# patrickltobing/cyclevae-vc

Measured on AMD Instinct MI355X. Metric: mcep_frames_per_sec_hu1024_ld32_cyc2, higher is better.
Workload: dtype f32 (every matrix product on exact fp32 operands: each operand carried as three fp16 limbs x = l0 + l1/2^11 + l2/2^22, six v_mfma_f32_32x32x16_f16 per product, f32 accumulate; dropped terms < 2^-33 of a product; gates, carried state, projection and outputs f32)

## Files before the change

cyclevae-vc_amd/csrc/cvae_exact3.h:

```cpp
#pragma once
#include <cvae_intrin.h>

struct Step6Params {
    const float* gx0;
    const float* w2s;
    float* hbuf;
    long mtot;
    float* hx;
    const float* wrec3;
    const float* afold3;
    const float* cfold;
    const float* bhn;
    const float* xt;
    int Tp, Cp;
    int B, Bp, H, T;
    unsigned* flags;
    int* status;
    long long* prof;
    const float* wyT;
    const float* dy;
    int Co;
    int rts;
    int want_f32;
    int exp;
    int backoff;
    const float* gx;
    long gx_bstride;
};

__global__ void k_prep_wrec3(const float* wrec2, float* wrec3, int H, int KPW, int* unfit) {
    const int nch = H >> 4, NB = H >> 3;
    const long idx = (long)blockIdx.x * blockDim.x + threadIdx.x;
    if (idx < (long)NB * 4 * KPW * 512) {
        const int e = (int)(idx & 7), lane = (int)((idx >> 3) & 63);
        const int s = (int)((idx >> 9) % KPW), wave = (int)(((idx >> 9) / KPW) & 3), c = (int)((idx >> 9) / KPW / 4);
        const int col = lane & 31, kh = lane >> 5, g = col >> 3, u = col & 7, j = 8 * c + u;
        const int k = 16 * (wave * KPW + s) + 8 * kh + e;
        float w = 0.0f;
        if (k < H) w = wrec2[((((long)(j >> 4) * 4 + g) * nch + (k >> 4)) * 16 + (j & 15)) * 16 + (k & 15)];
        unsigned short l0, l1, l2;
        cvae_split3_f16(w, l0, l1, l2);
        cvae_flag_unfit(unfit, w);
        unsigned short* dst = (unsigned short*)wrec3 + ((((long)c * 4 + wave) * KPW + s) * 3) * 512 + lane * 8 + e;
        dst[0] = l0;
        dst[512] = l1;
        dst[1024] = l2;
    }
}

__global__ void k_prep_wrec3_l2b(const float* wrec2, unsigned char* w2s, int H, int KPW) {
    const int nch = H >> 4, NB = H >> 3;
    const long idx = (long)blockIdx.x * blockDim.x + threadIdx.x;
    if (idx < (long)NB * 4 * KPW * 512) {
        const int e = (int)(idx & 7), lane = (int)((idx >> 3) & 63);
        const int s = (int)((idx >> 9) % KPW), wave = (int)(((idx >> 9) / KPW) & 3), c = (int)((idx >> 9) / KPW / 4);
        const int col = lane & 31, kh = lane >> 5, g = col >> 3, u = col & 7, j = 8 * c + u;
        const int k = 16 * (wave * KPW + s) + 8 * kh + e;
        float w = 0.0f;
        if (k < H) w = wrec2[((((long)(j >> 4) * 4 + g) * nch + (k >> 4)) * 16 + (j & 15)) * 16 + (k & 15)];
        unsigned short l0, l1;
        unsigned char l2;
        cvae_split3_f16b8(w, l0, l1, l2);
        w2s[idx] = l2;
    }
}

__global__ void k_prep_afold3l(const float* afold, float* afold3, int H, int Kfe, int KFW, int* unfit) {
    const int NB = H >> 3;
    const long idx = (long)blockIdx.x * blockDim.x + threadIdx.x;
    if (idx < (long)NB * 4 * KFW * 512) {
        const int e = (int)(idx & 7), lane = (int)((idx >> 3) & 63);
        const int s = (int)((idx >> 9) % KFW), wave = (int)(((idx >> 9) / KFW) & 3), c = (int)((idx >> 9) / KFW / 4);
        const int col = lane & 31, kh = lane >> 5, g = col >> 3, u = col & 7;
        const int k = 16 * (wave * KFW + s) + 8 * kh + e;
        const float w = (g < 3 && k < Kfe) ? afold[(long)(g * H + 8 * c + u) * Kfe + k] : 0.0f;
        unsigned short l0, l1, l2;
        cvae_split3_f16(w, l0, l1, l2);
        cvae_flag_unfit(unfit, w);
        unsigned short* dst = (unsigned short*)afold3 + ((((long)c * 4 + wave) * KFW + s) * 3) * 512 + lane * 8 + e;
        dst[0] = l0;
        dst[512] = l1;
        dst[1024] = l2;
    }
}

__device__ __forceinline__ f32x16 cvae_zero16() {
    f32x16 z;
#pragma unroll
    for (int q = 0; q < 16; ++q) z[q] = 0.0f;
    return z;
}

template <int KPW, int KFW, int LIMBS = 3, bool W2S = false>
__global__ __launch_bounds__(256, 1) void k_gru_steps_v6(Step6Params p) {
    constexpr int RS = 40;
    constexpr float S1 = 1.0f / 2048.0f;
#ifndef CVAE_V6_RD
#define CVAE_V6_RD 8
#endif
    constexpr int RD0 = W2S ? 5 : CVAE_V6_RD;
    constexpr int RD = KPW < RD0 ? KPW : RD0;
    constexpr bool HOIST = KFW == 0;
    constexpr int RF = HOIST ? 1 : (W2S && KFW > 3 ? 3 : KFW);
    constexpr int RW = KPW < 4 ? KPW : 4;
    const int tid = threadIdx.x, wave = cvae_uniform(tid >> 6), lane = tid & 63, lc = lane & 31, kh = lane >> 5;
    const int H = p.H, NB = H >> 3, nrt = p.Bp >> 5;
    const int rts = p.rts;
    int c, ti;
    cvae_block_map((int)blockIdx.x, NB, rts, (p.exp & 2) != 0, c, ti);
    const int s_lo = wave * KPW;
    float* red = (float*)CVAE_SMEM;
    float* hsh = red + 4 * 32 * RS;
    unsigned short* hl = (unsigned short*)(hsh + 32 * 8);
    float* wfl = hsh + 32 * 8 + 384;
    const int row = tid >> 3, u = tid & 7, j = 8 * c + u;
    const unsigned mtot = (unsigned)p.mtot;
    const cvae_buf hb = cvae_make_buf(p.hbuf, (unsigned)((long)(H >> 4) * p.mtot * 64));
    const cvae_buf xb_ = cvae_make_buf(p.hx, (unsigned)((long)(H >> 4) * p.mtot * 80));
    const unsigned tstride = mtot >> 5;
    const unsigned voff = (unsigned)kh * 512u + (unsigned)lc * 16u, voff2 = 2048u + (unsigned)kh * 256u + (unsigned)lc * 8u;
    f32x4 w0[KPW], w1[KPW], w2[LIMBS == 3 && !W2S ? KPW : 1];
#pragma unroll
    for (int s = 0; s < KPW; ++s) {
        const float* src = p.wrec3 + ((((long)c * 4 + wave) * KPW + s) * 3) * 256 + lane * 4;
        w0[s] = *(const f32x4*)src;
        w1[s] = *(const f32x4*)(src + 256);
        if constexpr (LIMBS == 3 && !W2S) w2[s] = *(const f32x4*)(src + 512);
    }
    {
        const float* src = p.afold3 + ((long)c * 4 + wave) * (KFW * 3 * 256);
        float* dst = wfl + wave * (KFW * LIMBS * 256);
#pragma unroll
        for (int s = 0; s < KFW; ++s)
#pragma unroll
            for (int m = 0; m < LIMBS; ++m)
                *(f32x4*)(dst + (s * LIMBS + m) * 256 + lane * 4) = *(const f32x4*)(src + (s * 3 + m) * 256 + lane * 4);
    }
    __syncthreads();
    const float* wfw = wfl + wave * (KFW * LIMBS * 256) + lane * 4;
    const float bhn = p.bhn[j];
    const float cf0 = HOIST ? 0.f : p.cfold[j], cf1 = HOIST ? 0.f : p.cfold[H + j], cf2 = HOIST ? 0.f : p.cfold[2 * H + j];
    const int ntile = ti < nrt ? (nrt - ti + rts - 1) / rts : 0, ntask = p.T * ntile;
    long long pc[4] = {0, 0, 0, 0};
    f32x4 x4[2 * RF];
    f32x2 x2[RF];
    const unsigned char* xw = nullptr;
    auto set_x = [&](int k) {
        const int tt = k / ntile, ii = ti + (k % ntile) * rts;
        xw = (const unsigned char*)p.xt + (((long)ii * p.Tp + tt) * (p.Cp >> 3) + 2 * (wave * KFW) + kh) * 1280;
    };
    auto load_x = [&](int s) {
        x4[2 * (s % RF)] = *(const f32x4*)(xw + s * 2560 + lc * 16);
        x4[2 * (s % RF) + 1] = *(const f32x4*)(xw + s * 2560 + 512 + lc * 16);
        if constexpr (LIMBS == 3) x2[s % RF] = *(const f32x2*)(xw + s * 2560 + 1024 + lc * 8);
    };
    float gq0 = 0.f, gq1 = 0.f, gq2 = 0.f;
    auto load_g = [&](int k) {
        const int tt = k / ntile, gr = (ti + (k % ntile) * rts) * 32 + row;
        if (gr < p.B) {
            const float* g = p.gx + (long)gr * p.gx_bstride + (long)tt * 3 * H + j;
            gq0 = g[0]; gq1 = g[H]; gq2 = g[2 * H];
        }
    };
    float hkeep0 = 0.f, hkeep1 = 0.f;
    const int backoff = (p.exp >> 8) ? (p.exp >> 8) - 1 : p.backoff;
    if constexpr (HOIST) {
        if (ntask > 0) load_g(0);
    } else if (ntask > 0) {
        set_x(0);
#pragma unroll
        for (int s = 0; s < RF; ++s) load_x(s);
    }
    unsigned fpre = 0u;
    for (int k = 0; k < ntask; ++k) {
        long long c0 = !W2S && p.prof ? cvae_clock() : 0;
        const int t = k / ntile, i = ti + (k % ntile) * rts;
        const unsigned row0 = (unsigned)(t * p.Bp + i * 32), tile0 = row0 >> 5;
        f32x16 a0 = cvae_zero16(), a1 = cvae_zero16(), a2 = cvae_zero16(), a3 = cvae_zero16();
#pragma unroll
        for (int s = 0; s < KFW; ++s) {
            const f32x4 l0 = x4[2 * (s % RF)], l1 = x4[2 * (s % RF) + 1];
            const f32x4 b0 = *(const f32x4*)(wfw + (s * LIMBS + 0) * 256);
            const f32x4 b1 = *(const f32x4*)(wfw + (s * LIMBS + 1) * 256);
            a0 = cvae_mfma_32x32x16_f16(l0, b0, a0);
            a1 = cvae_mfma_32x32x16_f16(l0, b1, a1);
            if constexpr (LIMBS == 3) {
                const f32x4 l2 = cvae_bf8x8_to_h8(x2[s % RF]);
                const f32x4 b2 = *(const f32x4*)(wfw + (s * LIMBS + 2) * 256);
                a2 = cvae_mfma_32x32x16_f16(l1, b1, a2);
                if constexpr (W2S) a2 = cvae_mfma_32x32x16_f16(l0, b2, a2);
                else a3 = cvae_mfma_32x32x16_f16(l0, b2, a3);
                a1 = cvae_mfma_32x32x16_f16(l1, b0, a1);
                a2 = cvae_mfma_32x32x16_f16(l2, b0, a2);
            } else {
                a2 = cvae_mfma_32x32x16_f16(l1, b0, a2);
            }
            cvae_sched_fence();
            if (s + RF < KFW) load_x(s + RF);
        }
        if (!W2S && p.prof) { const long long c1 = cvae_clock(); pc[0] += c1 - c0; c0 = c1; }
        const bool pre_ok = ntile > 1 && k > 0 && cvae_wave_all(fpre >= (unsigned)t);
        if (t > 0 && !pre_ok) {
            unsigned spins = 0;
            if (ntile == 1)
                for (int q = 0; q < backoff; ++q) cvae_sleep_64();
            for (;;) {
                unsigned f = (unsigned)t;
                if (lane < 2 * KPW && 2 * s_lo + lane < NB) f = cvae_atomic_load_agent(p.flags + (long)i * NB + 2 * s_lo + lane);
                if (cvae_wave_all(f >= (unsigned)t)) break;
                cvae_sleep();
                if (++spins > (1u << 22)) {
                    p.status[0] = 2;
                    break;
                }
            }
        }
        cvae_compiler_fence();
        if (!W2S && p.prof) { const long long c1 = cvae_clock(); pc[1] += c1 - c0; c0 = c1; }
        const int grow = i * 32 + row;
        const bool live = grow < p.B;
        const bool keep1 = ntile == 2 && (k & 1);
        float gxr = HOIST ? gq0 : cf0, gxz = HOIST ? gq1 : cf1, gxn = HOIST ? gq2 : cf2, hold = keep1 ? hkeep1 : hkeep0;
        auto gate_inputs = [&]() {
            if (live) {
                if (t == 0 && p.gx0) {
                    const float* g0p = p.gx0 + (long)grow * 3 * H + j;
                    gxr += g0p[0]; gxz += g0p[H]; gxn += g0p[2 * H];
                } else if (t == 0 && p.dy) cvae_t0_fix(p.wyT, p.dy, p.Co, H, j, grow, gxr, gxz, gxn);
                if (t == 0) {
                    hold = cvae_buf_load_f1_sc1(hb, (unsigned)(row * 64 + (j & 15) * 4), ((unsigned)(j >> 4) * mtot + row0) * 64u);
                } else if (ntile > 2) {
                    const unsigned so = ((unsigned)(j >> 4) * tstride + tile0) * 2560u, okh = (unsigned)((j >> 3) & 1);
                    const unsigned vo = okh * 512u + (unsigned)(row * 16 + (u >> 1) * 4);
                    const int sh = (u & 1) * 16;
                    const unsigned q0 = __builtin_bit_cast(unsigned, cvae_buf_load_f1_sc1(xb_, vo, so));
                    const unsigned q1 = __builtin_bit_cast(unsigned, cvae_buf_load_f1_sc1(xb_, vo, so + 1024u));
                    float third = 0.0f;
                    if constexpr (LIMBS == 3) {
                        const unsigned q2 = __builtin_bit_cast(unsigned, cvae_buf_load_f1_sc1(xb_, 2048u + okh * 256u + (unsigned)(row * 8 + (u >> 2) * 4), so));
                        third = cvae_bf8_to_f32((unsigned char)(q2 >> ((u & 3) * 8))) * (S1 / CVAE_L2_SCALE);
                    }
                    hold = cvae_f16_bits_to_f32((unsigned short)(q0 >> sh)) + (cvae_f16_bits_to_f32((unsigned short)(q1 >> sh)) + third) * S1;
                }
            }
        };
        if constexpr (KPW >= 32) gate_inputs();
        f32x4 hc[2 * RD];
        f32x2 hb2[RD];
        const unsigned tsel = (p.exp & 1) ? (unsigned)i : tile0;
        auto load_h = [&](int s) {
            const unsigned so = ((unsigned)(s_lo + s) * tstride + tsel) * 2560u;
            hc[2 * (s % RD)] = cvae_buf_load_f4(xb_, voff, so);
            hc[2 * (s % RD) + 1] = cvae_buf_load_f4(xb_, voff, so + 1024u);
            if constexpr (LIMBS == 3) hb2[s % RD] = cvae_buf_load_f2(xb_, voff2, so);
        };
        f32x2 w2r[W2S ? RW : 1];
        const float* w2base = W2S ? p.w2s + ((long)c * 4 + wave) * KPW * 128 + lane * 2 : nullptr;
        auto load_w2 = [&](int s) { w2r[s % RW] = *(const f32x2*)(w2base + s * 128); };
        if constexpr (W2S) {
#pragma unroll
            for (int s = 0; s < RW; ++s) load_w2(s);
        }
#pragma unroll
        for (int s = 0; s < RD; ++s) load_h(s);
        if constexpr (KPW < 32) gate_inputs();
#pragma unroll
        for (int s = 0; s < KPW; ++s) {
            const f32x4 l0 = hc[2 * (s % RD)], l1 = hc[2 * (s % RD) + 1];
            a0 = cvae_mfma_32x32x16_f16(l0, w0[s], a0);
            a1 = cvae_mfma_32x32x16_f16(l0, w1[s], a1);
            if constexpr (LIMBS == 3) {
                const f32x4 l2 = cvae_bf8x8_to_h8(hb2[s % RD]);
                a2 = cvae_mfma_32x32x16_f16(l1, w1[s], a2);
                if constexpr (W2S) a2 = cvae_mfma_32x32x16_f16(l0, cvae_bf8x8_to_h8(w2r[s % RW]), a2);
                else a3 = cvae_mfma_32x32x16_f16(l0, w2[s], a3);
                a1 = cvae_mfma_32x32x16_f16(l1, w0[s], a1);
                a2 = cvae_mfma_32x32x16_f16(l2, w0[s], a2);
            } else {
                a2 = cvae_mfma_32x32x16_f16(l1, w0[s], a2);
            }
            cvae_sched_fence();
            if (s + RD < KPW) load_h(s + RD);
            if constexpr (W2S) { if (s + RW < KPW) load_w2(s + RW); }
        }
        cvae_sched_fence();
        const int xmode = HOIST ? 0 : (p.exp >> 5) & 3;
        if constexpr (HOIST) {
            if (k + 1 < ntask) load_g(k + 1);
        } else {
            if (k + 1 < ntask) set_x(k + 1);
            if (k + 1 < ntask && (xmode == 0 || (xmode == 2 && wave != 0))) {
#pragma unroll
                for (int s = 0; s < RF; ++s) load_x(s);
            }
        }
#pragma unroll
        for (int q = 0; q < 16; ++q)
            red[(wave * 32 + (q & 3) + 8 * (q >> 2) + 4 * kh) * RS + lc] =
                LIMBS == 3 ? a0[q] + (a1[q] + (a2[q] + a3[q]) * S1) * S1 : a0[q] + (a1[q] + a2[q]) * S1;
        if (!W2S && p.prof) { const long long c1 = cvae_clock(); pc[2] += c1 - c0; c0 = c1; }
        __syncthreads();
        {
            float hn_ = 0.0f;
            if (live) {
                float sg[4];
#pragma unroll
                for (int g = 0; g < 4; ++g)
                    sg[g] = red[(0 * 32 + row) * RS + g * 8 + u] + red[(1 * 32 + row) * RS + g * 8 + u] +
                            red[(2 * 32 + row) * RS + g * 8 + u] + red[(3 * 32 + row) * RS + g * 8 + u];
                const float rg = cvae_sigmoid_fast(gxr + sg[0]);
                const float zg = cvae_sigmoid_fast(gxz + sg[1]);
                const float ng = cvae_tanh_fast(gxn + sg[2] + rg * (sg[3] + bhn));
                hn_ = ng + zg * (hold - ng);
            }
            if (keep1) hkeep1 = hn_; else hkeep0 = hn_;
            hsh[row * 8 + u] = hn_;
            unsigned short l0, l1;
            unsigned char l2;
            cvae_split3_f16b8(hn_, l0, l1, l2);
            hl[row * 8 + u] = l0;
            hl[256 + row * 8 + u] = l1;
            ((unsigned char*)(hl + 512))[row * 8 + u] = l2;
        }
        __syncthreads();
        if (tid < 64) {
            const unsigned so = ((unsigned)(c >> 1) * tstride + tile0 + (unsigned)(p.Bp >> 5)) * 2560u;
            cvae_buf_store_f4_sc1(xb_, (unsigned)(c & 1) * 512u + (unsigned)(tid & 31) * 16u, so + (unsigned)(tid >> 5) * 1024u,
                                  *(const f32x4*)(hl + tid * 8));
            if (LIMBS == 3 && tid < 32)
                cvae_buf_store_f2_sc1(xb_, 2048u + (unsigned)(c & 1) * 256u + (unsigned)tid * 8u, so, *(const f32x2*)(hl + 512 + tid * 4));
            cvae_drain_vmem();
            cvae_wave_barrier();
            if (tid == 0) cvae_atomic_store_agent(p.flags + (long)i * NB + c, (unsigned)(t + 1));
        } else if (tid < 128 && p.want_f32) {
            const int l = tid - 64, r = l >> 1, half = l & 1;
            *(f32x4*)(p.hbuf + (((long)(c >> 1) * p.mtot + row0 + p.Bp + r) * 16 + (c & 1) * 8 + half * 4)) =
                *(const f32x4*)(hsh + r * 8 + half * 4);
        }
        if constexpr (!HOIST) {
            if (k + 1 < ntask && (xmode == 1 || (xmode == 2 && wave == 0))) {
#pragma unroll
                for (int s = 0; s < RF; ++s) load_x(s);
            }
        }
        if (ntile > 1 && k + 1 < ntask) {
            const int kn = k + 1, tn = kn / ntile, in_ = ti + (kn % ntile) * rts;
            fpre = (unsigned)tn;
            if (tn > 0 && lane < 2 * KPW && 2 * s_lo + lane < NB)
                fpre = cvae_atomic_load_agent(p.flags + (long)in_ * NB + 2 * s_lo + lane);
        }
        if (!W2S && p.prof) { const long long c1 = cvae_clock(); pc[3] += c1 - c0; c0 = c1; }
    }
    if (p.prof && tid == 64 * ((p.exp >> 2) & 3))
        for (int q = 0; q < 4; ++q) p.prof[(long)blockIdx.x * 4 + q] = pc[q];
}

struct Out6Params {
    const float* hx;
    long mtot;
    const float* wo3;
    const float* bo2;
    int H, Bp, T, B, ncell, Co, clamp_from;
    float clamp_min;
    float* out[CVAE_MAX_CELLS];
};

__global__ void k_prep_wo3(const float* wo2, float* wo3, int H, int Cop, int NT, int* unfit) {
    const int nk = H >> 4;
    const long idx = (long)blockIdx.x * blockDim.x + threadIdx.x;
    if (idx < (long)NT * nk * 512) {
        const int e = (int)(idx & 7), lane = (int)((idx >> 3) & 63), s = (int)((idx >> 9) % nk), n = (int)((idx >> 9) / nk);
        const int col = 32 * n + (lane & 31), k = 16 * s + 8 * (lane >> 5) + e;
        const float w = col < Cop ? wo2[(long)col * H + k] : 0.0f;
        unsigned short l0, l1, l2;
        cvae_split3_f16(w, l0, l1, l2);
        cvae_flag_unfit(unfit, w);
        unsigned short* dst = (unsigned short*)wo3 + (((long)n * nk + s) * 3) * 512 + lane * 8 + e;
        dst[0] = l0;
        dst[512] = l1;
        dst[1024] = l2;
    }
}

template <int KPW>
__global__ __launch_bounds__(256) void k_outproj_v6(Out6Params p) {
    constexpr float S1 = 1.0f / 2048.0f;
    constexpr int RS = 36;
    const int tid = threadIdx.x, wave = cvae_uniform(tid >> 6), lane = tid & 63, lc = lane & 31, kh = lane >> 5;
    const int nk = p.H >> 4, nt32 = p.Bp >> 5;
    const int n = blockIdx.y;
    const long tile = (long)nt32 + blockIdx.x;
    float* red = (float*)CVAE_SMEM;
    const long tstride = p.mtot >> 5;
    f32x16 a0 = cvae_zero16(), a1 = cvae_zero16(), a2 = cvae_zero16(), a3 = cvae_zero16();
    constexpr int RD = KPW < 4 ? KPW : 4;
    f32x4 ha[2 * RD], wb[3 * RD];
    f32x2 hb[RD];
    auto load = [&](int s) {
        const int sg = wave * KPW + s;
        const unsigned char* hp = (const unsigned char*)p.hx + ((long)sg * tstride + tile) * 2560;
        ha[2 * (s % RD)] = *(const f32x4*)(hp + kh * 512 + lc * 16);
        ha[2 * (s % RD) + 1] = *(const f32x4*)(hp + 1024 + kh * 512 + lc * 16);
        hb[s % RD] = *(const f32x2*)(hp + 2048 + kh * 256 + lc * 8);
        const float* wp = p.wo3 + (((long)n * nk + sg) * 3) * 256 + lane * 4;
#pragma unroll
        for (int m = 0; m < 3; ++m) wb[3 * (s % RD) + m] = *(const f32x4*)(wp + m * 256);
    };
    const bool has_k = wave * KPW < nk;
    if (has_k) {
#pragma unroll
        for (int s = 0; s < RD; ++s) load(s);
#pragma unroll
        for (int s = 0; s < KPW; ++s) {
            const f32x4 l0 = ha[2 * (s % RD)], l1 = ha[2 * (s % RD) + 1], l2 = cvae_bf8x8_to_h8(hb[s % RD]);
            const f32x4 w0 = wb[3 * (s % RD)], w1 = wb[3 * (s % RD) + 1], w2 = wb[3 * (s % RD) + 2];
            a0 = cvae_mfma_32x32x16_f16(l0, w0, a0);
            a1 = cvae_mfma_32x32x16_f16(l0, w1, a1);
            a2 = cvae_mfma_32x32x16_f16(l1, w1, a2);
            a3 = cvae_mfma_32x32x16_f16(l0, w2, a3);
            a1 = cvae_mfma_32x32x16_f16(l1, w0, a1);
            a2 = cvae_mfma_32x32x16_f16(l2, w0, a2);
            cvae_sched_fence();
            if (s + RD < KPW) load(s + RD);
        }
    }
#pragma unroll
    for (int q = 0; q < 16; ++q)
        red[(wave * 32 + (q & 3) + 8 * (q >> 2) + 4 * kh) * RS + lc] = a0[q] + (a1[q] + (a2[q] + a3[q]) * S1) * S1;
    __syncthreads();
    {
        const int r = tid >> 3;
        const long m = (long)blockIdx.x * 32 + r;
        const int t = (int)(m / p.Bp), b = (int)(m - (long)t * p.Bp);
        if (b < p.ncell * p.B) {
            const int cell = b / p.B, bb = b - cell * p.B;
            float* orow = p.out[cell] + ((long)bb * p.T + t) * p.Co;
#pragma unroll
            for (int jj = 0; jj < 4; ++jj) {
                const int cl = (tid & 7) + 8 * jj, col = 32 * n + cl;
                if (col < p.Co) {
                    float v = red[(0 * 32 + r) * RS + cl] + red[(1 * 32 + r) * RS + cl] + red[(2 * 32 + r) * RS + cl] +
                              red[(3 * 32 + r) * RS + cl] + p.bo2[col];
                    if (p.clamp_from >= 0 && col >= p.clamp_from) v = fmaxf(v, p.clamp_min);
                    orow[col] = v;
                }
            }
        }
    }
}

__global__ void k_selftest_occupy(long long cycles, int lds_words) {
    float* occupy_lds = (float*)CVAE_SMEM;
    for (int i = threadIdx.x; i < lds_words; i += blockDim.x) occupy_lds[i] = (float)i;
    __syncthreads();
    const long long t0 = cvae_clock();
    float acc = 0.f;
    int guard = 0;
    while (cvae_clock() - t0 < cycles && ++guard < (1 << 28)) {
        acc += occupy_lds[(threadIdx.x * 33 + guard) % (lds_words > 0 ? lds_words : 1)];
        cvae_sleep();
    }
    if (acc == -1.0f) occupy_lds[0] = acc;
}

__global__ void k_selftest_limbs(const float* x, float* y, long n) {
    const long i0 = 8 * ((long)blockIdx.x * blockDim.x + threadIdx.x);
    if (i0 + 8 > n) return;
    unsigned short l0[8], l1[8];
    unsigned char b[8];
#pragma unroll
    for (int e = 0; e < 8; ++e) cvae_split3_f16b8(x[i0 + e], l0[e], l1[e], b[e]);
    unsigned w0 = 0, w1 = 0;
#pragma unroll
    for (int e = 0; e < 4; ++e) {
        w0 |= (unsigned)b[e] << (8 * e);
        w1 |= (unsigned)b[4 + e] << (8 * e);
    }
    const f32x2 raw = (f32x2){__builtin_bit_cast(float, w0), __builtin_bit_cast(float, w1)};
    const f32x4 h8 = cvae_bf8x8_to_h8(raw);
#pragma unroll
    for (int e = 0; e < 8; ++e) {
        const float pair = h8[e >> 1];
        const unsigned bits = __builtin_bit_cast(unsigned, pair);
        const unsigned short hb = (unsigned short)((e & 1) ? bits >> 16 : bits & 0xffffu);
        y[i0 + e] = cvae_f16_bits_to_f32(l0[e]) + cvae_f16_bits_to_f32(l1[e]) * (1.0f / 2048.0f) +
                    cvae_f16_bits_to_f32(hb) * (1.0f / 4194304.0f);
    }
}
```

cyclevae-vc_amd/csrc/cvae_lib.hip:

```cpp
#include <cvae_intrin.h>

#include <stdarg.h>
#include <stdio.h>
#include <stdlib.h>
#include <string.h>

#include <atomic>
#include <map>
#include <mutex>
#include <new>
#include <utility>
#include <vector>

#include "cvae_kernels.h"
#include "cvae_train_kernels.h"
#include "cvae_deep.h"
#include "cyclevae_hip.h"

namespace {

thread_local char g_err[512] = "";

enum OptId {
    OPT_V6_LIMBS_H64, OPT_NO_LL, OPT_MAX_RT, OPT_LL_BACKOFF, OPT_EXP, OPT_GEMM_FORCE, OPT_GEMM_LOG, OPT_TRAIN_OLD_GEMM,
// ... 23 lines not shown
    {"coop_launch", 0},
    {"v6_limbs_h2048", 3},
    {"v6_w2s_h64", 0},
    {"step_col_tiles", 0},
    {"train_profile", 0},
    {"train_xmap", 0},
    {"masks_on_side", 1},
    {"v6_backoff", -1},
    {"train_bwd_backoff", -1},
    {"ll_row_pad", 0},
    {"gemm_min_depth", 128},
    {"train_bwd_geom", -1},
    {"bwd_w3_l1_h64", 0},
    {"train_fwd_geom", -1},
    {"train_fwd_backoff", -1},
    {"exact_range_at", 65504},
};

struct ProfEvents {
    std::vector<hipEvent_t> start, stop;
    std::vector<int> rows, cin;
    size_t used = 0;
};
enum { TPROF_FWD = 0, TPROF_BWD = 1, TPROF_GEMM = 2, TPROF_WGRAD = 3, TPROF_CLASSES = 4 };
struct TrainProfEvents {
    std::vector<hipEvent_t> start, stop;
    std::vector<int> cls;
    std::vector<double> flop;
    size_t used = 0;
};
struct SideDone { const void* scratch; hipEvent_t ev; };

}

struct cvae_ctx {
    int32_t* status_sink = nullptr;
    long draw_row0 = 0, draw_rows = 0, draw_frames = 0, draw_parts = 1;
    long opt[OPT_COUNT];
    ProfEvents prof;
    TrainProfEvents tprof;
    hipStream_t side = nullptr;
    SideDone side_done[8] = {};
    hipEvent_t side_ready = nullptr, side_join = nullptr, side_last = nullptr;
    int side_cap = 0;
    hipEvent_t mask_fork = nullptr, mask_join = nullptr;
    unsigned side_evict = 0;
    std::map<const void*, std::pair<int, unsigned long>> train_var;
    unsigned long train_var_tick = 0;
    std::map<const void*, bool> image_unfit;
    int range_serial = 0;
    std::atomic<unsigned> ll_train_launch{1u};
};

namespace {

thread_local cvae_ctx* tl_ctx = nullptr;
inline cvae_ctx& cx() { return *tl_ctx; }
inline long opt(OptId i) { return tl_ctx->opt[i]; }
struct CtxScope {
    cvae_ctx* prev;
    explicit CtxScope(cvae_ctx* c) : prev(tl_ctx) {
        tl_ctx = c;
        g_cvae_coop_launch = (int)c->opt[OPT_COOP_LAUNCH];
    }
    ~CtxScope() { tl_ctx = prev; }
};

int fail(int code, const char* fmt, ...) {
    va_list ap;
    va_start(ap, fmt);
    vsnprintf(g_err, sizeof(g_err), fmt, ap);
    va_end(ap);
    return code;
}

#define CVAE_ENTER(c)                                                          \
    if (!(c)) return fail(-1, "null context (cvae_ctx_create)");               \
    CtxScope cvae_scope_(c)
#define CVAE_ENTER_SZ(c)                                                       \
    if (!(c)) {                                                                \
        (void)fail(-1, "null context (cvae_ctx_create)");                      \
        return 0;                                                              \
    }                                                                          \
    CtxScope cvae_scope_(c)

#define CVAE_HIP_OK(expr)                                                                         \
    do {                                                                                          \
        hipError_t e_ = (expr);                                                                   \
        if (e_ != hipSuccess) return fail(-3, "%s failed: %s", #expr, hipGetErrorString(e_));     \
    } while (0)

inline long up(long x, long m) { return (x + m - 1) / m * m; }
inline int clamp_dim(int v) { return v < 0 ? -1 : (v & ~CVAE_CLAMP_LAPLACE); }
inline float clamp_floor(int v) { return v >= 0 && (v & CVAE_CLAMP_LAPLACE) ? -7.2543288692621097f : -13.815510557964274f; }
inline unsigned nblk(long n, int per) { return (unsigned)((n + per - 1) / per); }

struct Dims {
    int C, Cp, Co, Cop, H, H3, ks, layers, R, pad, cl[3], cw, tot, Kfe, nch, KFW;
};

int make_dims(const cvae_net_desc* d, Dims* o) {
    if (!d) return fail(-1, "null net descriptor");
    if (d->layers < 1 || d->layers > 3) return fail(-1, "layers (reference dilation_size) must be 1, 2 or 3, got %d", d->layers);
    if (d->kernel_size < 1 || d->kernel_size % 2 == 0) return fail(-1, "kernel_size must be odd, got %d", d->kernel_size);
    if (d->hidden < 16 || d->hidden % 16) return fail(-1, "hidden must be a positive multiple of 16, got %d", d->hidden);
    if (d->in_dim < 1 || d->out_dim < 1) return fail(-1, "bad in_dim/out_dim %d/%d", d->in_dim, d->out_dim);
    if (d->layers == 3 && d->kernel_size != 3)
        return fail(-1, "layers == 3 needs kernel_size == 3: a front-end of kernel_size^3 >= 125 frames is not supported, got kernel_size %d",
                    d->kernel_size);
    if (d->layers == 3 && d->hidden % 64)
        return fail(-1, "layers == 3 needs hidden to be a multiple of 64, got %d", d->hidden);
    o->C = d->in_dim;
    o->Cp = (int)up(d->in_dim, 8);
    o->Co = d->out_dim;
    o->Cop = (int)up(d->out_dim, 16);
    o->H = d->hidden;
    o->H3 = 3 * d->hidden;
    o->ks = d->kernel_size;
    o->layers = d->layers;
    o->R = 1;
    o->cl[0] = o->cl[1] = o->cl[2] = 0;
    for (int i = 0; i < o->layers; ++i) {
        o->R *= o->ks;
        o->cl[i] = o->R * o->C;
    }
    o->pad = (o->R - 1) / 2;
    o->cw = o->R * o->C;
    o->tot = o->cw + o->Co;
    o->Kfe = (int)up((long)o->R * o->Cp, 16);
    o->nch = o->H / 16;
    o->KFW = (o->Kfe / 16 + 3) / 4;
    return 0;
}

int make_train_dims(const cvae_net_desc* d, Dims* o) {
    if (int rc = make_dims(d, o)) return rc;
    if (o->layers != 2)
        return fail(-1, "training is implemented for layers (reference dilation_size) == 2 only, got %d (eval and conversion run 1..3)", o->layers);
    return 0;
}

struct FoldScratch { long ma, mb, ba, bb, total; };
inline long fold_m_size(const Dims& m, int n) { return (long)m.cl[n] * (m.cl[n] / m.C) * m.C; }
inline FoldScratch fold_scratch(const Dims& m) {
    FoldScratch f;
    f.ma = 0;
    f.mb = fold_m_size(m, m.layers - 1);
    f.ba = f.mb + (m.layers > 1 ? fold_m_size(m, m.layers - 2) : 0);
    f.bb = f.ba + m.cw;
    f.total = f.bb + (m.layers > 1 ? m.cl[m.layers - 2] : 0) + 64;
    return f;
}

struct V6Inst { int H, KFW, limbs; bool w2s; void (*fn)(Step6Params); };
const V6Inst g_v6_inst[] = {
    {1024, 8, 3, false, k_gru_steps_v6<16, 8>},       {1024, 6, 3, false, k_gru_steps_v6<16, 6>},
    {1024, 3, 3, false, k_gru_steps_v6<16, 3>},       {1024, 2, 3, false, k_gru_steps_v6<16, 2>},
    {2048, 8, 3, true, k_gru_steps_v6<32, 8, 3, true>}, {2048, 11, 3, true, k_gru_steps_v6<32, 11, 3, true>},
    {2048, 8, 2, false, k_gru_steps_v6<32, 8, 2>},    {2048, 11, 2, false, k_gru_steps_v6<32, 11, 2>},
    {64, 3, 3, false, k_gru_steps_v6<1, 3>},          {64, 2, 3, false, k_gru_steps_v6<1, 2>},          {64, 1, 3, false, k_gru_steps_v6<1, 1>},
    {64, 3, 3, true, k_gru_steps_v6<1, 3, 3, true>},  {64, 2, 3, true, k_gru_steps_v6<1, 2, 3, true>},  {64, 1, 3, true, k_gru_steps_v6<1, 1, 3, true>},
    {64, 3, 2, false, k_gru_steps_v6<1, 3, 2>},       {64, 2, 2, false, k_gru_steps_v6<1, 2, 2>},       {64, 1, 2, false, k_gru_steps_v6<1, 1, 2>},
};
const int V6H_MIN_KFW = 12;
const V6Inst g_v6h_inst[] = {
    {1024, 0, 3, false, k_gru_steps_v6<16, 0>},
    {2048, 0, 3, true, k_gru_steps_v6<32, 0, 3, true>},
    {64, 0, 3, false, k_gru_steps_v6<1, 0>},          {64, 0, 3, true, k_gru_steps_v6<1, 0, 3, true>},  {64, 0, 2, false, k_gru_steps_v6<1, 0, 2>},
};
struct Fused16Inst { int H, KFW; void (*v5)(Step3Params); void (*v4)(Step3Params); };
const Fused16Inst g_fused16_inst[] = {
    {1024, 8, k_gru_steps_v5<16, 8>, k_gru_steps_v4<16, 8>}, {1024, 6, k_gru_steps_v5<16, 6>, k_gru_steps_v4<16, 6>},
    {64, 2, k_gru_steps_v5<1, 2>, k_gru_steps_v4<1, 2>},     {64, 1, k_gru_steps_v5<1, 1>, k_gru_steps_v4<1, 1>},
};
struct Out6Inst { int H; void (*fn)(Out6Params); };
const Out6Inst g_out6_inst[] = {{1024, k_outproj_v6<16>}, {2048, k_outproj_v6<32>}, {64, k_outproj_v6<1>}};

inline int exact3_kpw(const Dims& m) { return m.H / 64; }
inline const V6Inst* find_v6(const Dims& m, int limbs = -1, bool w2s = false) {
    for (const V6Inst& i : g_v6_inst)
        if (i.H == m.H && i.KFW == m.KFW && (limbs < 0 || (i.limbs == limbs && i.w2s == w2s))) return &i;
    return nullptr;
}
inline const Fused16Inst* find_fused16(const Dims& m) {
    for (const Fused16Inst& i : g_fused16_inst)
        if (i.H == m.H && i.KFW == m.KFW) return &i;
    return nullptr;
}
inline const V6Inst* find_v6h(const Dims& m, int limbs = -1, bool w2s = false) {
    if (m.KFW < V6H_MIN_KFW) return nullptr;
    for (const V6Inst& i : g_v6h_inst)
        if (i.H == m.H && (limbs < 0 || (i.limbs == limbs && i.w2s == w2s))) return &i;
    return nullptr;
}
inline bool exact3_fused(const Dims& m) { return find_v6(m) != nullptr; }
inline bool exact3_ok(const Dims& m) { return exact3_fused(m) || find_v6h(m) != nullptr; }
inline int v6_limbs(const Dims& m) {
    return (m.H == 64 && opt(OPT_V6_LIMBS_H64) == 2) || (m.H == 2048 && opt(OPT_V6_LIMBS_H2048) == 2) ? 2 : 3;
}
inline bool v6_w2s(const Dims& m) { return v6_limbs(m) == 3 && (m.H == 2048 || (m.H == 64 && opt(OPT_V6_W2S_H64))); }

struct Prep {
    long afold, afold3, afold_h, afold_t, cfold, wrec, wrec2, wrec_h, wrec_t, wrec_l2b, bhn, wyT, wo, bo, wo2, bo2, wo3, sin_w, sin_b, sout_w,
        sout_b, range, total;
};

Prep prep_layout(const Dims& m, bool sin, bool sout) {
    Prep p;
    long o = 0;
    auto take = [&](long n) { long r = o; o += up(n, 64); return r; };
    p.afold = take((long)m.H3 * m.Kfe);
    p.afold3 = take((long)m.nch * 4 * m.KFW * 3 * 256);
    p.afold_h = take((long)m.nch * 4 * ((m.KFW + 1) / 2) * 6 * 256);
    p.cfold = take(m.H3);
    p.wrec = take((long)(m.H / 4) * m.nch * 256);
    p.wrec2 = take((long)m.nch * 4 * m.nch * 256);
    p.wrec_h = take((long)m.nch * 4 * (m.H / 32) * 2 * 256);
    p.wrec_t = exact3_ok(m) ? take((long)(m.H / 8) * 4 * exact3_kpw(m) * 3 * 256) : -1;
    p.afold_t = exact3_fused(m) ? take((long)(m.H / 8) * 4 * m.KFW * 3 * 256) : -1;
    p.wrec_l2b = exact3_ok(m) ? take((long)(m.H / 8) * 4 * exact3_kpw(m) * 128) : -1;
    p.bhn = take(m.H);
    p.wyT = take((long)m.H3 * m.Co);
    p.wo = take((long)m.Cop * m.H);
    p.bo = take(m.Cop);
    p.wo2 = take((long)m.Cop * m.H);
    p.bo2 = take(m.Cop);
    p.wo3 = exact3_ok(m) ? take((long)((m.Cop + 31) / 32) * (m.H / 16) * 3 * 256) : -1;
    p.sin_w = sin ? take((long)m.C * m.C) : -1;
    p.sin_b = sin ? take(m.C) : -1;
    p.sout_w = sout ? take((long)m.Co * m.Co) : -1;
    p.sout_b = sout ? take(m.Co) : -1;
    p.range = take(64);
    p.total = o;
    return p;
}

struct Work {
    long status, xnp, xs, xs_plane, xt, xt_slack, gx, hbuf, hs, y, dy, gx0, prof, flags, total;
    int Bp, Tp, prof_blocks;
    long mtot;
};

inline int eval_row_pad(const Dims& m, int Brows) {
    return Brows <= 3 ? 16 : (exact3_ok(m) || Brows > 16 ? (int)up(Brows, 32) : 16);
}

Work work_layout(const Dims& m, int Brows, int T) {
    Work w;
    w.Bp = eval_row_pad(m, Brows);
    w.Tp = T + 2 * m.pad;
    w.mtot = (long)(T + 1) * w.Bp;
    long o = 0;
    auto take = [&](long n) { long r = o; o += up(n, 64); return r; };
    w.status = take(64);
    w.xnp = take((long)Brows * w.Tp * m.Cp + 64L * m.KFW + 64);
    w.xs_plane = up((long)Brows * w.Tp * m.Cp + 64L * m.KFW + 64, 8);
    w.xs = take(w.xs_plane);
    w.xt_slack = (64L * m.KFW / 8 + 2) * 640 + 64;
    w.xt = exact3_fused(m) && w.Bp % 32 == 0 ? take(((long)w.Bp * w.Tp * m.Cp * 5 / 2 + w.xt_slack) / 2 + 8) : -1;
    w.gx = take((long)Brows * w.Tp * m.H3);
    w.hbuf = take((long)m.nch * w.mtot * 16);
    w.hs = take((long)m.nch * w.mtot * 24);
    w.y = take((long)T * w.Bp * m.Cop);
    w.dy = take((long)w.Bp * m.Co);
    w.gx0 = take((long)w.Bp * m.H3);
    w.prof_blocks = 256;
    w.prof = take(w.prof_blocks * 8L);
    w.flags = take((long)(w.Bp / 16) * m.nch);
    w.total = o;
    return w;
}

inline int row_tiles_per_block(int cus, int per_tile, int ntiles) {
    int rts = per_tile > 0 ? cus / per_tile : 1;
    rts = rts < 1 ? 1 : (rts > ntiles ? ntiles : rts);
    if (opt(OPT_MAX_RT) >= 1 && opt(OPT_MAX_RT) < rts) rts = (int)opt(OPT_MAX_RT);
    return rts;
}

struct PassFacts {
    bool h_in, y_last, h_last, many_draws;
};
enum { PRO_ROWS = 0, PRO_DRAWS = 1, PRO_TILES = 2 };
enum { PROJ_GEMM = 0, PROJ_FUSED = 1, PROJ_V6 = 2 };
struct EvalPlan {
    int form;
    void (*k6)(Step6Params);
    void (*k5)(Step3Params);
    void (*k4)(Step3Params);
    void (*kout6)(Out6Params);
    int rts;
    int backoff;
    bool limbs;
    bool pairs;
    bool gx0_ready;
    bool want_f32;
    int prologue, proj;
};

inline int plain_projection(const Dims& m, bool y_last) {
    const int ntn = m.Cop / 16;
    return !y_last && (ntn == 1 || ntn == 4 || ntn == 8) ? PROJ_FUSED : PROJ_GEMM;
}

inline bool generic_resident(const Dims& m, int cus) { return cus <= 0 || m.H / 4 <= cus; }

EvalPlan plan_eval_pass(const Dims& m, int Brows, int T, int flags, int cus, bool unfit, const PassFacts& f) {
    EvalPlan pn;
    memset(&pn, 0, sizeof(pn));
    if (unfit) flags &= ~CVAE_FLAG_SPLIT_F16;
    const int Bp = eval_row_pad(m, Brows);
    const long mtot = (long)(T + 1) * Bp;
    const bool persistent = (flags & CVAE_FLAG_PERSISTENT) && T > 1, generic = (flags & CVAE_FLAG_GENERIC_STEP) != 0;
    const bool hoisted = (flags & CVAE_FLAG_HOISTED_FRONTEND) != 0, exact = persistent && (flags & CVAE_FLAG_EXACT3) && !generic;
    const V6Inst* i6 = find_v6(m, v6_limbs(m), v6_w2s(m));
    const V6Inst* i6h = find_v6h(m, v6_limbs(m), v6_w2s(m));
    const Fused16Inst* i16 = find_fused16(m);
    if (exact && Brows <= 3 && T < 65536 && m.H % 64 == 0 && m.H <= 1024 && cus >= m.H / 4 && !opt(OPT_NO_LL)) {
        pn.form = CVAE_EVAL_LL;
        pn.backoff = opt(OPT_LL_BACKOFF) >= 0 ? (int)opt(OPT_LL_BACKOFF) : (Brows == 1 ? 22 : 20);
    } else if (exact && !unfit && !hoisted && i6 && Bp % 32 == 0 && cus >= m.H / 8 && (long)m.nch * mtot * 80 < (1L << 31)) {
        pn.form = CVAE_EVAL_V6;
        pn.k6 = i6->fn;
        pn.rts = row_tiles_per_block(cus, m.H / 8, Bp / 32);
        pn.backoff = opt(OPT_V6_BACKOFF) >= 0 ? (int)opt(OPT_V6_BACKOFF) : (m.H == 1024 ? (m.KFW <= 6 ? 8 : 2) : 0);
    } else if (exact && !unfit && !hoisted && i6h && Bp % 32 == 0 && cus >= m.H / 8 && (long)m.nch * mtot * 80 < (1L << 31)) {
        pn.form = CVAE_EVAL_V6H;
        i6 = i6h;
        pn.k6 = i6h->fn;
        pn.rts = row_tiles_per_block(cus, m.H / 8, Bp / 32);
        pn.backoff = opt(OPT_V6_BACKOFF) >= 0 ? (int)opt(OPT_V6_BACKOFF) : 0;
    } else if (persistent && !generic && (m.H == 1024 || m.H == 64) && cus >= m.nch && (long)m.nch * mtot * 64 < (1L << 31)) {
        pn.form = hoisted || !i16 ? CVAE_EVAL_V2 : ((flags & CVAE_FLAG_SPLIT_F16) ? CVAE_EVAL_V5 : CVAE_EVAL_V4);
        if (i16) pn.k5 = i16->v5, pn.k4 = i16->v4;
        pn.rts = row_tiles_per_block(cus, m.nch, Bp / 16);
    } else {
        pn.form = persistent && generic_resident(m, cus) ? CVAE_EVAL_GENERIC : CVAE_EVAL_PER_STEP;
    }
    const bool v6f = pn.form == CVAE_EVAL_V6, v6 = v6f || pn.form == CVAE_EVAL_V6H;
    pn.limbs = v6 || pn.form == CVAE_EVAL_V5;
    pn.pairs = !v6 && (flags & CVAE_FLAG_SPLIT_F16);
    pn.gx0_ready = v6 && !f.h_in;
    pn.want_f32 = v6 && (i6->limbs != 3 || f.y_last || f.h_last || (opt(OPT_EXP) & 16));
    pn.prologue = v6f ? PRO_TILES : (f.many_draws ? PRO_DRAWS : PRO_ROWS);
    if (!f.y_last && v6 && i6->limbs == 3) {
        pn.proj = PROJ_V6;
        for (const Out6Inst& o : g_out6_inst)
            if (o.H == m.H) pn.kout6 = o.fn;
    } else {
        pn.proj = plain_projection(m, f.y_last);
    }
    return pn;
}

bool prof_begin(hipStream_t st, int rows = 0, int cin = 0) {
    if (cx().prof.used == cx().prof.start.size()) {
        hipEvent_t a, b;
        if (hipEventCreate(&a) != hipSuccess || hipEventCreate(&b) != hipSuccess) return false;
        cx().prof.start.push_back(a);
        cx().prof.stop.push_back(b);
        cx().prof.rows.push_back(0);
        cx().prof.cin.push_back(0);
    }
    cx().prof.rows[cx().prof.used] = rows;
    cx().prof.cin[cx().prof.used] = cin;
    return hipEventRecord(cx().prof.start[cx().prof.used], st) == hipSuccess;
}
void prof_end(hipStream_t st) {
    (void)hipEventRecord(cx().prof.stop[cx().prof.used], st);
    cx().prof.used++;
}

struct TrainProf {
    hipStream_t st;
    bool on;
    TrainProf(hipStream_t st_, int cls, double flop) : st(st_), on(false) {
        if (!opt(OPT_TRAIN_PROFILE)) return;
        if (cx().tprof.used == cx().tprof.start.size()) {
            hipEvent_t a, b;
            if (hipEventCreate(&a) != hipSuccess || hipEventCreate(&b) != hipSuccess) return;
            cx().tprof.start.push_back(a); cx().tprof.stop.push_back(b); cx().tprof.cls.push_back(0); cx().tprof.flop.push_back(0.0);
        }
        cx().tprof.cls[cx().tprof.used] = cls;
        cx().tprof.flop[cx().tprof.used] = flop;
        on = hipEventRecord(cx().tprof.start[cx().tprof.used], st) == hipSuccess;
    }
    void end() {
        if (!on) return;
        (void)hipEventRecord(cx().tprof.stop[cx().tprof.used], st);
        cx().tprof.used++;
        on = false;
    }
    ~TrainProf() { end(); }
};

__global__ void k_clear_words(int32_t* p, int n) {
    if ((int)threadIdx.x < n) p[threadIdx.x] = 0;
}
inline hipError_t clear_words(void* p, int n, hipStream_t st) {
    hipLaunchKernelGGL((k_clear_words), dim3(1), dim3(64), 0, st, (int32_t*)p, n);
    return hipGetLastError();
}

int cu_count() {
    static int cached[16] = {};
    int dev = 0, n = 0;
    if (hipGetDevice(&dev) != hipSuccess) return 0;
    if (dev >= 0 && dev < 16 && cached[dev] > 0) return cached[dev];
    if (hipDeviceGetAttribute(&n, hipDeviceAttributeMultiprocessorCount, dev) != hipSuccess) return 0;
    if (dev >= 0 && dev < 16) cached[dev] = n;
    return n;
}

inline bool image_known_unfit(const float* P) {
    auto it = cx().image_unfit.find((const void*)P);
    return it != cx().image_unfit.end() && it->second;
}
inline void range_params(ProParams& pp, int* ws_status, bool limbs, bool new_call, const float* P, const Prep& pl) {
    if (new_call) {
        cx().range_serial += 1;
        if (cx().range_serial <= 0) cx().range_serial = 1;
    }
    long at = opt(OPT_EXACT_RANGE_AT);
    at = at < 1 ? 1 : (at > 65504 ? 65504 : at);
    pp.range_at = (float)at;
    pp.image_unfit = (const int*)(P + pl.range);
    if (cx().status_sink) {
        pp.range_word = limbs ? cx().status_sink + CVAE_STATUS_RANGE_WORD : nullptr;
        pp.range_epoch = nullptr;
        pp.range_val = CVAE_STATUS_RANGE;
    } else {
        pp.range_word = limbs ? ws_status + CVAE_WS_RANGE_WORD : nullptr;
        pp.range_epoch = new_call ? ws_status + CVAE_WS_RANGE_EPOCH : nullptr;
        pp.range_val = cx().range_serial;
    }
}

struct Cell {
    const cvae_pass_input* in;
    const float* y_in;
    const float* h_in;
    float* trj_out;
    float* y_last;
    float* h_last;
};


inline int last_slot(const cvae_pass_input* in, int T) { return in->frames > 0 && in->frames < T ? in->frames : T; }

struct PassRows {
    const Cell* cells;
    int ncell, B, T, Bp;
    long mtot;
};

int check_cells(const Dims& m, const PassRows& r) {
    const Cell* cells = r.cells;
    const int ncell = r.ncell, B = r.B, T = r.T;
    if (ncell > CVAE_MAX_CELLS) return fail(-1, "at most %d stacked cells per pass", CVAE_MAX_CELLS);
    for (int c = 0; c < ncell; ++c) {
        const cvae_pass_input* in = cells[c].in;
        const int w_in = in->seg0.width + (in->lat ? in->lat_dim : in->seg1.width);
        if (w_in != m.C) return fail(-1, "cell %d: pass input width %d != in_dim %d", c, w_in, m.C);
        if (in->frames < 0 || in->frames > T) return fail(-1, "cell %d: frames %d outside [0, T=%d]", c, in->frames, T);
        if (in->ctx_before < 0 || in->ctx_after < 0 || in->draw_frame0 < 0 || in->eps_draw_stride < 0)
            return fail(-1, "cell %d: negative window context / draw origin", c);
        if ((in->ctx_before || in->ctx_after || in->draw_frame0) && B != 1)
            return fail(-1, "cell %d: windows of a longer utterance (ctx_before / ctx_after / draw_frame0) are single-row cells, B=%d", c, B);
    }
    return 0;
}

struct ProTargets {
    int shape;
    float* xnp;
    float* dy;
    float* slot0;
    unsigned* zero_words;
    int nzero;
    int* zero_status;
    int zero_status_n;
    int* ws_status;
// ... 828 lines not shown
```

Measured before the change: 1.295 million.

## Pin recurrent weights in AGPRs, prefetch frontend weights, compile out profiling

In the H=1024 exact-3 GRU step kernel, the recurrent weight limbs are forced into accumulator registers via an inline-asm constraint. This frees ordinary vector registers. The freed registers are used to double-buffer the folded frontend weights from shared memory, so each sub-step's operands are loaded ahead of its MFMAs, and for small KFW the first block is loaded before the flag wait. Profiling clock reads become a template parameter instead of a runtime check, which removes branches and counter registers from the production kernel. The spin backoff defaults for H=1024 are also retuned. The added register pressure and the AGPR-to-VGPR moves could cause spills or extra copies.

```diff
diff --git a/cyclevae-vc_amd/csrc/cvae_exact3.h b/cyclevae-vc_amd/csrc/cvae_exact3.h
--- a/cyclevae-vc_amd/csrc/cvae_exact3.h
+++ b/cyclevae-vc_amd/csrc/cvae_exact3.h
@@ -1,5 +1,11 @@
 #pragma once
 #include <cvae_intrin.h>
+
+#if defined(__HIP_DEVICE_COMPILE__)
+#define CVAE_V6_IN_AGPR(x) asm volatile("" : "+a"(x))
+#else
+#define CVAE_V6_IN_AGPR(x) ((void)0)
+#endif
 
 struct Step6Params {
     const float* gx0;
@@ -91,8 +97,9 @@
     return z;
 }
 
-template <int KPW, int KFW, int LIMBS = 3, bool W2S = false>
+template <int KPW, int KFW, int LIMBS = 3, bool W2S = false, bool PROF = false>
 __global__ __launch_bounds__(256, 1) void k_gru_steps_v6(Step6Params p) {
+    static_assert(!(W2S && PROF), "no phase counters in the W2S form: no registers to spare");
     constexpr int RS = 40;
     constexpr float S1 = 1.0f / 2048.0f;
 #ifndef CVAE_V6_RD
@@ -101,6 +108,13 @@
     constexpr int RD0 = W2S ? 5 : CVAE_V6_RD;
     constexpr int RD = KPW < RD0 ? KPW : RD0;
     constexpr bool HOIST = KFW == 0;
+#ifndef CVAE_V6_WACC
+#define CVAE_V6_WACC 1
+#endif
+#ifndef CVAE_V6_FPRE
+#define CVAE_V6_FPRE 1
+#endif
+    constexpr bool WACC = CVAE_V6_WACC && KPW == 16 && LIMBS == 3 && !W2S;
     constexpr int RF = HOIST ? 1 : (W2S && KFW > 3 ? 3 : KFW);
     constexpr int RW = KPW < 4 ? KPW : 4;
     const int tid = threadIdx.x, wave = cvae_uniform(tid >> 6), lane = tid & 63, lc = lane & 31, kh = lane >> 5;
@@ -127,6 +141,14 @@
         w1[s] = *(const f32x4*)(src + 256);
         if constexpr (LIMBS == 3 && !W2S) w2[s] = *(const f32x4*)(src + 512);
     }
+    if constexpr (WACC) {
+#pragma unroll
+        for (int s = 0; s < KPW; ++s) {
+            CVAE_V6_IN_AGPR(w0[s]);
+            CVAE_V6_IN_AGPR(w1[s]);
+            CVAE_V6_IN_AGPR(w2[s]);
+        }
+    }
     {
         const float* src = p.afold3 + ((long)c * 4 + wave) * (KFW * 3 * 256);
         float* dst = wfl + wave * (KFW * LIMBS * 256);
@@ -141,7 +163,7 @@
     const float bhn = p.bhn[j];
     const float cf0 = HOIST ? 0.f : p.cfold[j], cf1 = HOIST ? 0.f : p.cfold[H + j], cf2 = HOIST ? 0.f : p.cfold[2 * H + j];
     const int ntile = ti < nrt ? (nrt - ti + rts - 1) / rts : 0, ntask = p.T * ntile;
-    long long pc[4] = {0, 0, 0, 0};
+    long long pc[PROF ? 4 : 1] = {};
     f32x4 x4[2 * RF];
     f32x2 x2[RF];
     const unsigned char* xw = nullptr;
@@ -162,6 +184,17 @@
             gq0 = g[0]; gq1 = g[H]; gq2 = g[2 * H];
         }
     };
+    constexpr bool FPRE = CVAE_V6_FPRE && !HOIST && LIMBS == 3 && !W2S && KPW <= 16;
+    constexpr bool FW0_EARLY = KFW <= 6;
+    f32x4 fw[FPRE ? 2 * LIMBS : 1];
+    auto load_fw = [&](int s) {
+#pragma unroll
+        for (int m = 0; m < LIMBS; ++m) fw[(s & 1) * LIMBS + m] = *(const f32x4*)(wfw + (s * LIMBS + m) * 256);
+    };
+    auto fw_op = [&](int s, int m) -> f32x4 {
+        if constexpr (FPRE) return fw[(s & 1) * LIMBS + m];
+        else return *(const f32x4*)(wfw + (s * LIMBS + m) * 256);
+    };
     float hkeep0 = 0.f, hkeep1 = 0.f;
     const int backoff = (p.exp >> 8) ? (p.exp >> 8) - 1 : p.backoff;
     if constexpr (HOIST) {
@@ -171,22 +204,29 @@
 #pragma unroll
         for (int s = 0; s < RF; ++s) load_x(s);
     }
+    if constexpr (FPRE && FW0_EARLY) { if (ntask > 0) load_fw(0); }
     unsigned fpre = 0u;
     for (int k = 0; k < ntask; ++k) {
-        long long c0 = !W2S && p.prof ? cvae_clock() : 0;
+        long long c0 = 0;
+        if constexpr (PROF) c0 = cvae_clock();
         const int t = k / ntile, i = ti + (k % ntile) * rts;
         const unsigned row0 = (unsigned)(t * p.Bp + i * 32), tile0 = row0 >> 5;
         f32x16 a0 = cvae_zero16(), a1 = cvae_zero16(), a2 = cvae_zero16(), a3 = cvae_zero16();
+        if constexpr (FPRE && !FW0_EARLY) load_fw(0);
 #pragma unroll
         for (int s = 0; s < KFW; ++s) {
             const f32x4 l0 = x4[2 * (s % RF)], l1 = x4[2 * (s % RF) + 1];
-            const f32x4 b0 = *(const f32x4*)(wfw + (s * LIMBS + 0) * 256);
-            const f32x4 b1 = *(const f32x4*)(wfw + (s * LIMBS + 1) * 256);
+            if constexpr (FPRE) {
+                if (s + 1 < KFW) load_fw(s + 1);
+                cvae_sched_fence();
+            }
+            const f32x4 b0 = fw_op(s, 0);
+            const f32x4 b1 = fw_op(s, 1);
             a0 = cvae_mfma_32x32x16_f16(l0, b0, a0);
             a1 = cvae_mfma_32x32x16_f16(l0, b1, a1);
             if constexpr (LIMBS == 3) {
                 const f32x4 l2 = cvae_bf8x8_to_h8(x2[s % RF]);
-                const f32x4 b2 = *(const f32x4*)(wfw + (s * LIMBS + 2) * 256);
+                const f32x4 b2 = fw_op(s, 2);
                 a2 = cvae_mfma_32x32x16_f16(l1, b1, a2);
                 if constexpr (W2S) a2 = cvae_mfma_32x32x16_f16(l0, b2, a2);
                 else a3 = cvae_mfma_32x32x16_f16(l0, b2, a3);
@@ -198,7 +238,7 @@
             cvae_sched_fence();
             if (s + RF < KFW) load_x(s + RF);
         }
-        if (!W2S && p.prof) { const long long c1 = cvae_clock(); pc[0] += c1 - c0; c0 = c1; }
+        if constexpr (PROF) { const long long c1 = cvae_clock(); pc[0] += c1 - c0; c0 = c1; }
         const bool pre_ok = ntile > 1 && k > 0 && cvae_wave_all(fpre >= (unsigned)t);
         if (t > 0 && !pre_ok) {
             unsigned spins = 0;
@@ -216,7 +256,7 @@
             }
         }
         cvae_compiler_fence();
-        if (!W2S && p.prof) { const long long c1 = cvae_clock(); pc[1] += c1 - c0; c0 = c1; }
+        if constexpr (PROF) { const long long c1 = cvae_clock(); pc[1] += c1 - c0; c0 = c1; }
         const int grow = i * 32 + row;
         const bool live = grow < p.B;
         const bool keep1 = ntile == 2 && (k & 1);
@@ -298,7 +338,7 @@
         for (int q = 0; q < 16; ++q)
             red[(wave * 32 + (q & 3) + 8 * (q >> 2) + 4 * kh) * RS + lc] =
                 LIMBS == 3 ? a0[q] + (a1[q] + (a2[q] + a3[q]) * S1) * S1 : a0[q] + (a1[q] + a2[q]) * S1;
-        if (!W2S && p.prof) { const long long c1 = cvae_clock(); pc[2] += c1 - c0; c0 = c1; }
+        if constexpr (PROF) { const long long c1 = cvae_clock(); pc[2] += c1 - c0; c0 = c1; }
         __syncthreads();
         {
             float hn_ = 0.0f;
@@ -349,10 +389,13 @@
             if (tn > 0 && lane < 2 * KPW && 2 * s_lo + lane < NB)
                 fpre = cvae_atomic_load_agent(p.flags + (long)in_ * NB + 2 * s_lo + lane);
         }
-        if (!W2S && p.prof) { const long long c1 = cvae_clock(); pc[3] += c1 - c0; c0 = c1; }
-    }
-    if (p.prof && tid == 64 * ((p.exp >> 2) & 3))
-        for (int q = 0; q < 4; ++q) p.prof[(long)blockIdx.x * 4 + q] = pc[q];
+        if constexpr (FPRE && FW0_EARLY) { if (k + 1 < ntask) load_fw(0); }
+        if constexpr (PROF) { const long long c1 = cvae_clock(); pc[3] += c1 - c0; c0 = c1; }
+    }
+    if constexpr (PROF) {
+        if (p.prof && tid == 64 * ((p.exp >> 2) & 3))
+            for (int q = 0; q < 4; ++q) p.prof[(long)blockIdx.x * 4 + q] = pc[q];
+    }
 }
 
 struct Out6Params {
diff --git a/cyclevae-vc_amd/csrc/cvae_lib.hip b/cyclevae-vc_amd/csrc/cvae_lib.hip
--- a/cyclevae-vc_amd/csrc/cvae_lib.hip
+++ b/cyclevae-vc_amd/csrc/cvae_lib.hip
@@ -199,22 +199,26 @@
     return f;
 }
 
-struct V6Inst { int H, KFW, limbs; bool w2s; void (*fn)(Step6Params); };
+struct V6Inst { int H, KFW, limbs; bool w2s; void (*fn)(Step6Params); void (*fn_prof)(Step6Params); };
+#define V6_PAIR(KPW, KFW, LIMBS) k_gru_steps_v6<KPW, KFW, LIMBS>, k_gru_steps_v6<KPW, KFW, LIMBS, false, true>
+#define V6_W2S(KPW, KFW) k_gru_steps_v6<KPW, KFW, 3, true>, nullptr
 const V6Inst g_v6_inst[] = {
-    {1024, 8, 3, false, k_gru_steps_v6<16, 8>},       {1024, 6, 3, false, k_gru_steps_v6<16, 6>},
-    {1024, 3, 3, false, k_gru_steps_v6<16, 3>},       {1024, 2, 3, false, k_gru_steps_v6<16, 2>},
-    {2048, 8, 3, true, k_gru_steps_v6<32, 8, 3, true>}, {2048, 11, 3, true, k_gru_steps_v6<32, 11, 3, true>},
-    {2048, 8, 2, false, k_gru_steps_v6<32, 8, 2>},    {2048, 11, 2, false, k_gru_steps_v6<32, 11, 2>},
-    {64, 3, 3, false, k_gru_steps_v6<1, 3>},          {64, 2, 3, false, k_gru_steps_v6<1, 2>},          {64, 1, 3, false, k_gru_steps_v6<1, 1>},
-    {64, 3, 3, true, k_gru_steps_v6<1, 3, 3, true>},  {64, 2, 3, true, k_gru_steps_v6<1, 2, 3, true>},  {64, 1, 3, true, k_gru_steps_v6<1, 1, 3, true>},
-    {64, 3, 2, false, k_gru_steps_v6<1, 3, 2>},       {64, 2, 2, false, k_gru_steps_v6<1, 2, 2>},       {64, 1, 2, false, k_gru_steps_v6<1, 1, 2>},
+    {1024, 8, 3, false, V6_PAIR(16, 8, 3)},  {1024, 6, 3, false, V6_PAIR(16, 6, 3)},
+    {1024, 3, 3, false, V6_PAIR(16, 3, 3)},  {1024, 2, 3, false, V6_PAIR(16, 2, 3)},
+    {2048, 8, 3, true, V6_W2S(32, 8)},       {2048, 11, 3, true, V6_W2S(32, 11)},
+    {2048, 8, 2, false, V6_PAIR(32, 8, 2)},  {2048, 11, 2, false, V6_PAIR(32, 11, 2)},
+    {64, 3, 3, false, V6_PAIR(1, 3, 3)},     {64, 2, 3, false, V6_PAIR(1, 2, 3)},          {64, 1, 3, false, V6_PAIR(1, 1, 3)},
+    {64, 3, 3, true, V6_W2S(1, 3)},          {64, 2, 3, true, V6_W2S(1, 2)},               {64, 1, 3, true, V6_W2S(1, 1)},
+    {64, 3, 2, false, V6_PAIR(1, 3, 2)},     {64, 2, 2, false, V6_PAIR(1, 2, 2)},          {64, 1, 2, false, V6_PAIR(1, 1, 2)},
 };
 const int V6H_MIN_KFW = 12;
 const V6Inst g_v6h_inst[] = {
-    {1024, 0, 3, false, k_gru_steps_v6<16, 0>},
-    {2048, 0, 3, true, k_gru_steps_v6<32, 0, 3, true>},
-    {64, 0, 3, false, k_gru_steps_v6<1, 0>},          {64, 0, 3, true, k_gru_steps_v6<1, 0, 3, true>},  {64, 0, 2, false, k_gru_steps_v6<1, 0, 2>},
-};
+    {1024, 0, 3, false, V6_PAIR(16, 0, 3)},
+    {2048, 0, 3, true, V6_W2S(32, 0)},
+    {64, 0, 3, false, V6_PAIR(1, 0, 3)},     {64, 0, 3, true, V6_W2S(1, 0)},               {64, 0, 2, false, V6_PAIR(1, 0, 2)},
+};
+#undef V6_PAIR
+#undef V6_W2S
 struct Fused16Inst { int H, KFW; void (*v5)(Step3Params); void (*v4)(Step3Params); };
 const Fused16Inst g_fused16_inst[] = {
     {1024, 8, k_gru_steps_v5<16, 8>, k_gru_steps_v4<16, 8>}, {1024, 6, k_gru_steps_v5<16, 6>, k_gru_steps_v4<16, 6>},
@@ -368,13 +372,13 @@
         pn.backoff = opt(OPT_LL_BACKOFF) >= 0 ? (int)opt(OPT_LL_BACKOFF) : (Brows == 1 ? 22 : 20);
     } else if (exact && !unfit && !hoisted && i6 && Bp % 32 == 0 && cus >= m.H / 8 && (long)m.nch * mtot * 80 < (1L << 31)) {
         pn.form = CVAE_EVAL_V6;
-        pn.k6 = i6->fn;
+        pn.k6 = (flags & CVAE_FLAG_STEP_TIMING) && i6->fn_prof ? i6->fn_prof : i6->fn;
         pn.rts = row_tiles_per_block(cus, m.H / 8, Bp / 32);
-        pn.backoff = opt(OPT_V6_BACKOFF) >= 0 ? (int)opt(OPT_V6_BACKOFF) : (m.H == 1024 ? (m.KFW <= 6 ? 8 : 2) : 0);
+        pn.backoff = opt(OPT_V6_BACKOFF) >= 0 ? (int)opt(OPT_V6_BACKOFF) : (m.H == 1024 ? (m.KFW > 6 ? 10 : (m.KFW == 6 ? 16 : 8)) : 0);
     } else if (exact && !unfit && !hoisted && i6h && Bp % 32 == 0 && cus >= m.H / 8 && (long)m.nch * mtot * 80 < (1L << 31)) {
         pn.form = CVAE_EVAL_V6H;
         i6 = i6h;
-        pn.k6 = i6h->fn;
+        pn.k6 = (flags & CVAE_FLAG_STEP_TIMING) && i6h->fn_prof ? i6h->fn_prof : i6h->fn;
         pn.rts = row_tiles_per_block(cus, m.H / 8, Bp / 32);
         pn.backoff = opt(OPT_V6_BACKOFF) >= 0 ? (int)opt(OPT_V6_BACKOFF) : 0;
     } else if (persistent && !generic && (m.H == 1024 || m.H == 64) && cus >= m.nch && (long)m.nch * mtot * 64 < (1L << 31)) {
```

Result: faster. 1.325 million (median of 6 runs) (+2.3%).
